# hsp-iit/roft

Measured on AMD Instinct MI355X. Metric: tracker frames/sec per object (640x480) + ADD-S vs CPU ref, higher is better.
Workload: dtype f64; 1 GPU; BASELINE config #4: 640x480, CV_32FC2 flow grid 1, 64 objects in total, 64 per GPU (sharded by object, no data-path collective; result rows all-gathered over RCCL at N > 1), masks+poses at 5 fps with 6-frame delay, flow-aided masks, re-sync and outlier rejection on, frames submitted in batches of at most 8; objects_per_gpu=64, objects_total=64, width=640, height=480, batch_frames=8, ranks=1, backend=nccl

## Files before the change

include/roft_engine.h:

```cpp
#ifndef ROFT_ENGINE_H
#define ROFT_ENGINE_H

#include <stddef.h>
#include <stdint.h>

#ifdef __cplusplus
extern "C" {
#endif

#define ROFT_ABI_VERSION 2

#define ROFT_OK 0
#define ROFT_ERR_INVALID (-1)
#define ROFT_ERR_DEVICE (-2)
#define ROFT_ERR_CAPACITY (-3)
#define ROFT_ERR_STATE (-4)

#define ROFT_FLOW_S16C2 11
#define ROFT_FLOW_F32C2 13

#define ROFT_MEAS_NONE 0
#define ROFT_MEAS_VELOCITY 1
#define ROFT_MEAS_POSE 2
#define ROFT_MEAS_POSE_VELOCITY 3
// ... 250 lines not shown
typedef struct roft_scene_renderer roft_scene_renderer;
int roft_scene_renderer_create(const roft_camera* cam, const roft_mesh* meshes, int n_meshes, int max_frames_per_call, int device,
                               roft_scene_renderer** out);
int roft_scene_renderer_destroy(roft_scene_renderer* r);
int roft_scene_render(roft_scene_renderer* r, const roft_scene_desc* desc, uint8_t* rgb_out, float* depth_out, int32_t* instance_out,
                      int32_t* triangle_out);
int roft_render_scene(const roft_camera* cam, const roft_mesh* meshes, int n_meshes, const roft_scene_desc* desc, uint8_t* rgb_out,
                      float* depth_out, int32_t* instance_out, int32_t* triangle_out);

int roft_debug_plan(const roft_config* cfg, const int* pose_valid, int n_frames, int* n_steps, int* n_corrections,
                    int* outlier, int* slots);
int roft_debug_probe_streams(roft_engine* e, double out[25]);
int roft_debug_sector_rate(int device, double* sectors_per_second);
int roft_debug_get_residency(roft_engine* e, unsigned long long out[32]);
int roft_debug_outlier_split(int mode);
int roft_debug_pose_errors_kernel_ms(double* ms_out);
int roft_debug_scene_kernel_ms(roft_scene_renderer* r, double ms_out[2]);
int roft_debug_get_dbg(roft_engine* e, int obj_id, long long out[32]);

#ifdef __cplusplus
}
#endif
#endif
```

roft_amd/_lib.py:

```python
import ctypes as C
import os
import subprocess

_HERE = os.path.dirname(os.path.abspath(__file__))
CSRC = os.path.join(_HERE, "csrc")
SO = os.environ.get("ROFT_LIB_SO") or os.path.join(CSRC, "libroft_hip.so")

OK = 0
FLOW_S16C2 = 11
FLOW_F32C2 = 13
MEAS_NONE, MEAS_VELOCITY, MEAS_POSE, MEAS_POSE_VELOCITY = 0, 1, 2, 3
MEM_HOST, MEM_DEVICE = 0, 1
RETAIN_FRAMES = 16
MAX_BATCH_FRAMES = 8
MAX_FLOW_CHASE = 30
RENDER_CONTRACT, RENDER_GL = 0, 1
ABI_VERSION = 2


class RoftError(RuntimeError):
    pass


class Camera(C.Structure):
# ... 73 lines not shown


SCENE_MAX_INSTANCES = 256

ABI_SYMBOLS = [
    "roft_last_error_string", "roft_device_count", "roft_abi_version", "roft_flow_measurement", "roft_kf_predict",
    "roft_skf_correct", "roft_skf_correct_points", "roft_mask_propagate", "roft_pose_process_noise", "roft_ukf_predict",
    "roft_ukf_correct", "roft_mesh_classify", "roft_render_depth", "roft_render_depth_mode", "roft_depth_likelihood", "roft_outlier_test",
    "roft_outlier_test_split", "roft_outlier_test_mode", "roft_default_config",
    "roft_default_object", "roft_engine_create", "roft_engine_destroy", "roft_object_add",
    "roft_frame_submit", "roft_frames_submit", "roft_engine_retain_frames", "roft_engine_get_stats", "roft_step", "roft_sync", "roft_get_state", "roft_get_outputs", "roft_get_mask",
    "roft_engine_enable_log", "roft_engine_get_log", "roft_engine_get_log_rows", "roft_engine_stream", "roft_engine_enable_timing",
    "roft_engine_get_timing", "roft_engine_get_batch_trace", "roft_default_of_params", "roft_optical_flow", "roft_flow_producer_create",
    "roft_flow_producer_destroy", "roft_flow_producer_run", "roft_flow_producer_sync", "roft_flow_producer_stream",
    "roft_debug_plan", "roft_debug_get_dbg", "roft_debug_probe_streams", "roft_debug_sector_rate",
    "roft_host_alloc", "roft_host_free", "roft_host_is_pinned", "roft_debug_get_residency", "roft_debug_outlier_split",
    "roft_pose_errors", "roft_engine_score_log", "roft_debug_pose_errors_kernel_ms",
    "roft_scene_renderer_create", "roft_scene_renderer_destroy", "roft_scene_render", "roft_render_scene", "roft_debug_scene_kernel_ms",
]
POSE_ERROR_ADD, POSE_ERROR_ADDS = 0, 1
NEWER_SYMBOLS = ("roft_pose_errors", "roft_engine_score_log", "roft_scene_renderer_create", "roft_scene_renderer_destroy", "roft_scene_render",
                 "roft_render_scene")


def build(force=False):
    srcs = [os.path.join(CSRC, f) for f in os.listdir(CSRC) if f.endswith((".hip", ".h"))]
    srcs.append(os.path.join(_HERE, "..", "include", "roft_engine.h"))
    stale = (not os.path.exists(SO)) or any(os.path.getmtime(s) > os.path.getmtime(SO) for s in srcs)
    if force or stale:
        jobs = str(min(8, os.cpu_count() or 1))
        r = subprocess.run(["make", "-C", CSRC, "-j", jobs, "libroft_hip.so"], capture_output=True, text=True)
# ... 103 lines not shown
```

roft_amd/csrc/engine.hip:

```cpp
#include "engine_internal.h"

namespace {
thread_local std::string g_last_error;
}

namespace roft {
namespace host {
int fail(int code, const std::string& msg)
{
    g_last_error = msg;
    return code;
}
}
}
const std::string& last_error() { return g_last_error; }

namespace roft {
int set_last_error(int code, const std::string& msg) { return fail(code, msg); }

int device_cu_count()
{
    static std::mutex mu;
    static std::vector<int> cus;
    int dev = 0;
// ... 536 lines not shown
    auto bail = [&](int code, const std::string& msg) { delete o; return fail(code, msg); };
    if (d->mesh.n_verts > 0 && d->mesh.n_tris > 0) {
        if (!d->mesh.verts || !d->mesh.tris) return bail(ROFT_ERR_INVALID, "mesh: null vertex or triangle array");
        for (size_t i = 0; i < (size_t)3 * d->mesh.n_tris; ++i)
            if (d->mesh.tris[i] < 0 || d->mesh.tris[i] >= d->mesh.n_verts)
                return bail(ROFT_ERR_INVALID, "mesh: triangle " + std::to_string(i / 3) + " refers to vertex " + std::to_string(d->mesh.tris[i]) +
                                                  " of " + std::to_string(d->mesh.n_verts));
        PreparedMesh pm;
        if (e->cfg.render_mode == ROFT_RENDER_CONTRACT) prepare_mesh(d->mesh.verts, d->mesh.n_verts, d->mesh.tris, d->mesh.n_tris, pm);
        hipError_t err = o->verts.ensure((size_t)3 * d->mesh.n_verts);
        if (err == hipSuccess) err = o->tris.ensure((size_t)3 * d->mesh.n_tris);
        if (err == hipSuccess && pm.closed) err = o->tri_flip.ensure((size_t)d->mesh.n_tris);
        if (err == hipSuccess) err = hipMemcpy(o->verts.p, d->mesh.verts, sizeof(float) * 3 * d->mesh.n_verts, hipMemcpyHostToDevice);
        if (err == hipSuccess) err = hipMemcpy(o->tris.p, pm.tris(d->mesh.tris), sizeof(int32_t) * 3 * d->mesh.n_tris, hipMemcpyHostToDevice);
        if (err == hipSuccess && pm.closed) err = hipMemcpy(o->tri_flip.p, pm.flip.data(), (size_t)d->mesh.n_tris, hipMemcpyHostToDevice);
        if (err != hipSuccess) return bail(ROFT_ERR_DEVICE, std::string("mesh upload: ") + hipGetErrorString(err));
        p.verts = o->verts.p; p.tris = o->tris.p;
        p.tri_flip = pm.closed ? o->tri_flip.p : nullptr;
        p.n_verts = d->mesh.n_verts; p.n_tris = d->mesh.n_tris;
    } else if (e->cfg.outlier_rejection && e->cfg.use_pose) {
        return bail(ROFT_ERR_INVALID, "outlier rejection needs a mesh");
    }
    ObjState* st = new ObjState();
    init_state(*st);
    for (int i = 0; i < 6; ++i) { st->v_mean[i] = d->v_mean0[i]; st->v_cov[i * 6 + i] = d->v_cov0_diag[i]; }
    PoseBelief b{};
    for (int i = 0; i < 13; ++i) b.mean[i] = d->p_mean0[i];
    for (int i = 0; i < 12; ++i) b.cov[i * 12 + i] = d->p_cov0_diag[i];
    st->belief[B_LIN0] = b;
    st->belief[B_LIN1] = b;
    st->belief[B_PRED] = st->belief[B_PRED + 1] = b;
    hipError_t err = hipMemcpy(e->arr.params.p + id, &p, sizeof(p), hipMemcpyHostToDevice);
    if (err == hipSuccess) err = hipMemcpy(e->arr.state.p + id, st, sizeof(ObjState), hipMemcpyHostToDevice);
// ... 13 lines not shown
```

roft_amd/csrc/engine_debug.hip:

```cpp
#include "engine_internal.h"


extern "C" int roft_debug_get_dbg(roft_engine* e, int id, long long out[32])
{
    if (!e || id < 0 || id >= (int)e->objs.size()) return ROFT_ERR_INVALID;
    if (roft_sync(e) != ROFT_OK) return ROFT_ERR_DEVICE;
    ObjState* st = new ObjState();
    hipError_t err = hipMemcpy(st, e->arr.state.p + id, sizeof(ObjState), hipMemcpyDeviceToHost);
    if (err == hipSuccess) std::memcpy(out, st->dbg, sizeof(long long) * 32);
    delete st;
    if (err == hipSuccess) err = hipMemset(reinterpret_cast<char*>(e->arr.state.p + id) + offsetof(ObjState, dbg), 0, sizeof(long long) * 32);
    return err == hipSuccess ? ROFT_OK : ROFT_ERR_DEVICE;
}

extern "C" int roft_debug_outlier_split(int mode)
{
    roft::set_outlier_split(mode);
    return ROFT_OK;
}

extern "C" int roft_debug_get_residency(roft_engine* e, unsigned long long out[32])
{
    if (!e || !out) return ROFT_ERR_INVALID;
    if (roft_sync(e) != ROFT_OK) return ROFT_ERR_DEVICE;
    if (hipMemcpy(out, e->arr.residency.p, sizeof(unsigned long long) * 32, hipMemcpyDeviceToHost) != hipSuccess) return ROFT_ERR_DEVICE;
    return hipMemset(e->arr.residency.p, 0, sizeof(unsigned long long) * 32) == hipSuccess ? ROFT_OK : ROFT_ERR_DEVICE;
}

extern "C" int roft_debug_sector_rate(int device, double* sectors_per_second)
{
    if (!sectors_per_second) return fail(ROFT_ERR_INVALID, "null output");
    HIP_TRY(hipSetDevice(device));
// ... 83 lines not shown
```

roft_amd/csrc/engine_internal.h:

```cpp
#pragma once

#include <hip/hip_runtime.h>

#include <algorithm>
#include <cfloat>
#include <chrono>
#include <cmath>
#include <cstdio>
#include <cstdlib>
#include <cstring>
#include <deque>
#include <map>
#include <mutex>
#include <string>
#include <vector>

#include "roft_device.h"
#include "mesh_class.h"
#include "batch_plan.h"

static_assert(roft::host::kPlanLanes == roft::kNumLin, "batch_plan.h plans for the engine's pose lanes");


namespace roft {
// ... 201 lines not shown
    Sched() { for (int& u : feat_use) u = -1; }
};

struct OwnedFlow {
    DevBuf<unsigned char> buf;
    int last_ref_frame = -1;
};

struct HostObject {
    Sched s;
    int stepped_slot = 0, stepped_lane = 0;
    std::vector<OwnedFlow*> owned;
    DevBuf<float> verts;
    DevBuf<int32_t> tris;
    DevBuf<uint8_t> tri_flip;
    ~HostObject() { for (auto* o : owned) delete o; }
};

struct StageFrame {
    std::vector<DevBuf<unsigned char>*> chunks;
    size_t cur = 0, used = 0;
    std::vector<std::pair<const void*, void*>> seen;
    StageFrame() = default;
    StageFrame(StageFrame&&) = default;
    StageFrame(const StageFrame&) = delete;
    ~StageFrame() { for (auto* c : chunks) delete c; }
};
constexpr size_t kStageChunk = (size_t)32 << 20;


// ... 127 lines not shown
```

roft_amd/csrc/engine_ops.hip:

```cpp
#include "engine_internal.h"

namespace {

struct OpCtx {
    std::mutex mu;
    hipStream_t stream = nullptr;
    Arrays arr;
    int W = 0, H = 0, ftype = 0, fgrid = 0, radius = 0;
    DevBuf<unsigned char> b0, b1, b2, b3, b4, b5, bflip;
    bool ready = false;

    int prepare(const roft_camera& cam, int ftype_, int fgrid_, float fscale, int radius_)
    {
        if (roft_device_count() <= 0) return fail(ROFT_ERR_DEVICE, "no HIP device (libroft_hip has no CPU path)");
        if (int rc = check_geometry(cam.width, cam.height)) return rc;
        HIP_TRY(hipSetDevice(0));
        (void)hipGetLastError();
        if (!stream) HIP_TRY(hipStreamCreateWithFlags(&stream, hipStreamNonBlocking));
        DevFlowFmt ff;
        ff.type = ftype_;
        ff.grid = std::max(fgrid_, 1);
        ff.cols = cam.width / ff.grid;
        ff.rows = cam.height / ff.grid;
        ff.scale = fscale;
// ... 398 lines not shown
    if (int rc = c.arr.ensure_zmerge(1, tpix)) return rc;
    auto restore = [&]() {
        a.cam = make_cam(*cam);
        a.tile_w = cam->width / a.cam.divider;
        a.tile_h = cam->height / a.cam.divider;
        a.max_verts = a.max_tris = 0;
    };
    for (size_t i = 0; i < (size_t)3 * mesh->n_tris; ++i)
        if (mesh->tris[i] < 0 || mesh->tris[i] >= mesh->n_verts) return fail(ROFT_ERR_INVALID, "mesh: a triangle refers to a vertex outside the vertex array");
    PreparedMesh pm;
    if (o_in.render_mode == ROFT_RENDER_CONTRACT) prepare_mesh(mesh->verts, mesh->n_verts, mesh->tris, mesh->n_tris, pm);
    if (int rc = to_dev(c.b0, mesh->verts, (size_t)3 * mesh->n_verts, c.stream)) return rc;
    if (int rc = to_dev(c.b1, pm.tris(mesh->tris), (size_t)3 * mesh->n_tris, c.stream)) return rc;
    if (pm.closed)
        if (int rc = to_dev(c.bflip, pm.flip.data(), (size_t)mesh->n_tris, c.stream)) return rc;
    ObjParams prm;
    std::memset(&prm, 0, sizeof(prm));
    prm.verts = reinterpret_cast<const float*>(c.b0.p);
    prm.tris = reinterpret_cast<const int32_t*>(c.b1.p);
    prm.tri_flip = pm.closed ? reinterpret_cast<const uint8_t*>(c.bflip.p) : nullptr;
    prm.n_verts = mesh->n_verts;
    prm.n_tris = mesh->n_tris;
    a.max_verts = mesh->n_verts;
    a.max_tris = mesh->n_tris;
    FrameCtrl fc;
    clear_ctrl(fc);
    fc.n_steps = 1;
    fc.outlier_step = 0;
    fc.cur_slot = B_LIN0;
    fc.lane = 0;
    fc.feat_read = 0;
    if (depth && mask) {
        std::vector<uint8_t> zero;
        if (int rc = to_dev(c.b2, mask, npix, c.stream)) return rc;
        if (int rc = to_dev(c.b3, depth, npix, c.stream)) return rc;
// ... 211 lines not shown
```

roft_amd/csrc/k_render.hip:

```cpp
#include <algorithm>
#include <atomic>

#include "plane_rank.h"
#include "raster.h"

namespace roft {

constexpr int kFeatThreads = 1024;

#ifdef ROFT_FEAT_PROFILE
#define FTICK(i) do { __syncthreads(); if (threadIdx.x == 0) { long long _t = wall_clock64(); a.state[obj].dbg[i] = _t - f_t0; f_t0 = _t; } } while (0)
#else
#define FTICK(i) do {} while (0)
#endif

template <bool LDS>
__global__ __launch_bounds__(kFeatThreads) void features_kernel(EngineArrays a, unsigned frames_packed)
{
    ROFT_RESIDENT(a, RK_FEATURES);
    extern __shared__ __attribute__((aligned(16))) unsigned char smem[];
    __shared__ int s_wave[16];
    __shared__ int s_chunk[kFeatThreads];
    const int obj = blockIdx.x;
    const FrameCtrl& c = frame_ctrl(a, (int)((frames_packed >> (4 * blockIdx.y)) & 15u), obj);
// ... 279 lines not shown
    const int alt = bx / parts, part = bx % parts, tid = threadIdx.x;
    ObjState& st = a.state[obj];
    PoseLane& pl = st.lane[lin];
    if (pl.pending_frame < 0) return;
    const FrameCtrl& c = frame_ctrl(a, pl.pending_frame, obj);
    const ObjParams& prm = a.params[obj];
    const PoseBelief& bl = st.belief[b_alt(lin, alt)];
    const RenderPose P = make_pose(bl.mean + 6, bl.mean + 9);
    const int d = a.cam.divider, tw = a.tile_w, th = a.tile_h;
    const float fx = (float)(a.cam.fx / d), fy = (float)(a.cam.fy / d), cx = (float)(a.cam.cx / d), cy = (float)(a.cam.cy / d);
    const int nv = prm.n_verts, nt = prm.n_tris;
    const bool cached = nv <= vcache_cap;
    float* s_v = reinterpret_cast<float*>(smem);
    uint32_t* s_z = reinterpret_cast<uint32_t*>(smem + (((size_t)vcache_cap * 12 + 15) & ~(size_t)15));
    uint64_t* s_k = reinterpret_cast<uint64_t*>(s_z);
    if (tid < 4) s_box[tid] = (tid < 2) ? INT32_MAX : -1;
    if (tid == 0) s_behind = 0;
#ifdef ROFT_FUSED_PROFILE
    long long u_t0 = wall_clock64();
    if (tid < 8 && bx < 4) st.dbg[bx * 8 + tid] = 0;
#endif
    __syncthreads();
    {
        int bi0 = INT32_MAX, bj0 = INT32_MAX, bi1 = -1, bj1 = -1;
        bool behind = false;
        constexpr int kVB = 4;
        for (int vb = tid; vb < nv; vb += kVB * kFusedThreads) {
          float vc[kVB][3];
#pragma unroll
          for (int k = 0; k < kVB; ++k) {
// ... 23 lines not shown
        for (int off = 32; off > 0; off >>= 1) {
            bi0 = min(bi0, __shfl_xor(bi0, off, 64)); bj0 = min(bj0, __shfl_xor(bj0, off, 64));
            bi1 = max(bi1, __shfl_xor(bi1, off, 64)); bj1 = max(bj1, __shfl_xor(bj1, off, 64));
        }
        if ((tid & 63) == 0) {
            atomicMin(&s_box[0], bi0); atomicMin(&s_box[1], bj0);
            atomicMax(&s_box[2], bi1); atomicMax(&s_box[3], bj1);
        }
    }
    __syncthreads();
    UTICK(0);
    const int i0 = min(s_box[0], tw - 1), i1 = s_box[2];
    int j0 = min(s_box[1], th - 1), j1 = s_box[3];
    int R = parts;
    if (!GL && split_tris && parts > 1 && i1 >= i0 && j1 >= j0 && i0 >= 0 && j0 >= 0) {
        const long long w_all = i1 - i0 + 1, rows_all = j1 - j0 + 1;
        for (R = 1; R < parts; ++R)
            if (parts % R == 0 && ((rows_all + R - 1) / R) * w_all <= (long long)win_cap) break;
    }
    const int G = parts / R, band = part / G, grp = part % G;
    const bool split = G > 1;
    if (j1 >= j0 && R > 1) {
        const int rows_all = j1 - j0 + 1, b0 = j0 + (int)((long long)rows_all * band / R), b1 = j0 + (int)((long long)rows_all * (band + 1) / R) - 1;
        j0 = b0;
        j1 = b1;
    }
    const int win_w = i1 - i0 + 1;
    const int fslot = (c.feat_read >= 0) ? c.feat_read : 0;
    const uint32_t* fpix = a.feat_pix + ((size_t)obj * kFeatRing + fslot) * a.feat_cap;
    const float* fdep = a.feat_depth + ((size_t)obj * kFeatRing + fslot) * a.feat_cap;
    const int n = st.n_feat[fslot];
    LikelihoodSum err;
    int cnt = 0;
    auto gl_resolve = [&](uint64_t key, int i, int j) -> float {
        const int32_t* tri = prm.tris + (size_t)3 * (uint32_t)key;
        const int v0 = tri[0], v1 = tri[1], v2 = tri[2];
        float x0, y0, z0, x1, y1, z1, x2, y2, z2;
        if (cached) {
// ... 2 lines not shown
            x2 = s_v[3 * v2]; y2 = s_v[3 * v2 + 1]; z2 = s_v[3 * v2 + 2];
        } else {
            project_vertex_gl(prm.verts + (size_t)3 * v0, P, fx, fy, cx, cy, x0, y0, z0);
            project_vertex_gl(prm.verts + (size_t)3 * v1, P, fx, fy, cx, cy, x1, y1, z1);
            project_vertex_gl(prm.verts + (size_t)3 * v2, P, fx, fy, cx, cy, x2, y2, z2);
        }
        return gl_linear_depth(gl_pixel_window_z(x0, y0, x1, y1, x2, y2, gl_vertex_window_z(z0), gl_vertex_window_z(z1),
                                                 gl_vertex_window_z(z2), (float)i + 0.5f, (float)j + 0.5f));
    };
    if (win_w > 0 && j1 >= j0 && i0 >= 0 && j0 >= 0) {
        const int rows = max(1, win_cap / win_w);
        for (int js = j0; js <= j1; js += rows) {
            const int je = min(j1, js + rows - 1), npx = win_w * (je - js + 1);
            if constexpr (GL) {
                for (int i = tid; i < npx; i += kFusedThreads) s_k[i] = kGlKeyClear;
            } else {
                for (int i = tid; i < npx; i += kFusedThreads) s_z[i] = 0x7F800000u;
            }
            __syncthreads();
            UTICK(1);
            ROFT_LDS uint32_t* const zw = pin_lds(s_z);
            auto store = [zw, i0, js, win_w](int i, int j, float z) {
                (void)__hip_atomic_fetch_min(zw + ((j - js) * win_w + (i - i0)), __float_as_uint(z), __ATOMIC_RELAXED, __HIP_MEMORY_SCOPE_WORKGROUP);
            };
            ROFT_LDS uint64_t* const zk = (ROFT_LDS uint64_t*)zw;
            auto store_key = [zk, i0, js, win_w](int i, int j, uint64_t key) {
                (void)__hip_atomic_fetch_min(zk + ((j - js) * win_w + (i - i0)), key, __ATOMIC_RELAXED, __HIP_MEMORY_SCOPE_WORKGROUP);
            };
            constexpr int kTB = 8;
            const uint8_t* const flips = (!GL && prm.tri_flip && !s_behind && nv < (1 << 30)) ? prm.tri_flip : nullptr;
            const int stride = G, first = grp;
            auto tri_of = [=](int slot) { return ((slot >> 6) * stride + first) * 64 + (slot & 63); };
            const int n_slots = split ? ((nt + 63) / 64 + stride - 1 - first) / stride * 64 : nt;
            for (int tb = tid; tb < n_slots; tb += kTB * kFusedThreads) {
              int idx[kTB][3];
#pragma unroll
              for (int k = 0; k < kTB; ++k) {
                  const int t = min(tri_of(min(tb + k * kFusedThreads, n_slots - 1)), nt - 1);
                  const int32_t* tri = prm.tris + (size_t)3 * t;
                  idx[k][0] = tri[0]; idx[k][1] = tri[1]; idx[k][2] = tri[2];
                  if (flips) idx[k][0] |= (1 + (int)flips[t]) << 30;
              }
#pragma unroll
              for (int k = 0; k < kTB; ++k) {
                if (tb + k * kFusedThreads >= n_slots || tri_of(tb + k * kFusedThreads) >= nt) break;
                const int cull_k = (int)((unsigned)idx[k][0] >> 30);
                const int v0 = idx[k][0] & 0x3FFFFFFF, v1 = idx[k][1], v2 = idx[k][2];
                float x0, y0, z0, x1, y1, z1, x2, y2, z2;
                if (cached) {
                    x0 = s_v[3 * v0]; y0 = s_v[3 * v0 + 1]; z0 = s_v[3 * v0 + 2];
                    x1 = s_v[3 * v1]; y1 = s_v[3 * v1 + 1]; z1 = s_v[3 * v1 + 2];
                    x2 = s_v[3 * v2]; y2 = s_v[3 * v2 + 1]; z2 = s_v[3 * v2 + 2];
                } else if constexpr (GL) {
                    project_vertex_gl(prm.verts + (size_t)3 * v0, P, fx, fy, cx, cy, x0, y0, z0);
                    project_vertex_gl(prm.verts + (size_t)3 * v1, P, fx, fy, cx, cy, x1, y1, z1);
                    project_vertex_gl(prm.verts + (size_t)3 * v2, P, fx, fy, cx, cy, x2, y2, z2);
                } else {
                    project_vertex(prm.verts + (size_t)3 * v0, P, fx, fy, cx, cy, x0, y0, z0);
                    project_vertex(prm.verts + (size_t)3 * v1, P, fx, fy, cx, cy, x1, y1, z1);
                    project_vertex(prm.verts + (size_t)3 * v2, P, fx, fy, cx, cy, x2, y2, z2);
                }
                if constexpr (GL) {
                    const uint64_t t = (uint32_t)tri_of(tb + k * kFusedThreads);
                    raster_projected_gl(x0, y0, z0, x1, y1, z1, x2, y2, z2, tw, th, js, je,
                                        [&](int i, int j, uint32_t qz) { store_key(i, j, ((uint64_t)qz << 32) | t); });
                } else {
                    raster_projected(x0, y0, z0, x1, y1, z1, x2, y2, z2, tw, th, js, je, cull_k, store);
                }
              }
            }
            __syncthreads();
            UTICK(2);
            if constexpr (!GL) if (split) {
                const size_t slab0 = (((size_t)lin * a.zmerge_slabs + (size_t)obj * parts + (size_t)band * G) * 2 + alt) * a.zmerge_stride;
                uint32_t* mine = a.zmerge + slab0 + (size_t)grp * 2 * a.zmerge_stride;
                int* arrivals = a.zcount + (((size_t)lin * a.n_obj + obj) * 2 + alt) * kMaxOutlierParts + band;
                for (int i = tid; i < npx; i += kFusedThreads)
                    __hip_atomic_store(&mine[i], s_z[i], __ATOMIC_RELAXED, __HIP_MEMORY_SCOPE_AGENT);
                __atomic_signal_fence(__ATOMIC_SEQ_CST);
                __builtin_amdgcn_s_waitcnt(0);
                __atomic_signal_fence(__ATOMIC_SEQ_CST);
                __syncthreads();
                if (tid == 0) {
                    const int before = __hip_atomic_fetch_add(arrivals, 1, __ATOMIC_RELAXED, __HIP_MEMORY_SCOPE_AGENT);
                    s_last = (before == G - 1) ? 1 : 0;
                    if (before == G - 1) __hip_atomic_store(arrivals, 0, __ATOMIC_RELAXED, __HIP_MEMORY_SCOPE_AGENT);
                }
                __syncthreads();
                if (!s_last) return;
                static_assert(kMaxOutlierParts <= 8, "eight slabs per pixel");
                const uint32_t* others = a.zmerge + slab0;
                const size_t slab_step = 2 * a.zmerge_stride;
                const uint32_t* op[7];
                {
                    int k = 0;
#pragma unroll
                    for (int p = 0; p < 8; ++p)
                        if (p < G && p != grp && k < 7) op[k++] = others + (size_t)p * slab_step;
                    for (; k < 7; ++k) op[k] = others;
                }
                for (int i = tid; i < npx; i += kFusedThreads) {
                    uint32_t m = s_z[i];
                    uint32_t v0, v1, v2, v3, v4, v5, v6;
                    switch (G - 1) {
                    case 1:
                        asm volatile("global_load_dword %0, %1, off sc1\n\ts_waitcnt vmcnt(0)" : "=&v"(v0) : "v"(op[0] + i) : "memory");
                        m = min(m, v0);
                        break;
                    case 2:
                        asm volatile("global_load_dword %0, %2, off sc1\n\tglobal_load_dword %1, %3, off sc1\n\ts_waitcnt vmcnt(0)"
                                     : "=&v"(v0), "=&v"(v1) : "v"(op[0] + i), "v"(op[1] + i) : "memory");
                        m = min(m, min(v0, v1));
                        break;
                    case 3:
                        asm volatile("global_load_dword %0, %3, off sc1\n\tglobal_load_dword %1, %4, off sc1\n\tglobal_load_dword %2, %5, off sc1\n\t"
                                     "s_waitcnt vmcnt(0)"
                                     : "=&v"(v0), "=&v"(v1), "=&v"(v2) : "v"(op[0] + i), "v"(op[1] + i), "v"(op[2] + i) : "memory");
                        m = min(min(m, v0), min(v1, v2));
                        break;
                    case 4:
                        asm volatile("global_load_dword %0, %4, off sc1\n\tglobal_load_dword %1, %5, off sc1\n\tglobal_load_dword %2, %6, off sc1\n\t"
                                     "global_load_dword %3, %7, off sc1\n\ts_waitcnt vmcnt(0)"
                                     : "=&v"(v0), "=&v"(v1), "=&v"(v2), "=&v"(v3) : "v"(op[0] + i), "v"(op[1] + i), "v"(op[2] + i), "v"(op[3] + i) : "memory");
                        m = min(m, min(min(v0, v1), min(v2, v3)));
                        break;
                    default:
                        asm volatile("global_load_dword %0, %7, off sc1\n\tglobal_load_dword %1, %8, off sc1\n\tglobal_load_dword %2, %9, off sc1\n\t"
                                     "global_load_dword %3, %10, off sc1\n\tglobal_load_dword %4, %11, off sc1\n\tglobal_load_dword %5, %12, off sc1\n\t"
                                     "global_load_dword %6, %13, off sc1\n\ts_waitcnt vmcnt(0)"
                                     : "=&v"(v0), "=&v"(v1), "=&v"(v2), "=&v"(v3), "=&v"(v4), "=&v"(v5), "=&v"(v6)
                                     : "v"(op[0] + i), "v"(op[1] + i), "v"(op[2] + i), "v"(op[3] + i), "v"(op[4] + i), "v"(op[5] + i), "v"(op[6] + i) : "memory");
                        m = min(min(m, v0), min(min(v1, v2), min(min(v3, v4), min(v5, v6))));
                        break;
                    case 0: break;
                    }
                    s_z[i] = m;
                }
                __syncthreads();
            }
            if (tile_dump) {
                float* tile = tile_dump + (size_t)alt * tw * th;
                if constexpr (GL) {
                    for (int i = tid; i < npx; i += kFusedThreads) {
                        const uint64_t key = s_k[i];
                        const int pi = i0 + i % win_w, pj = js + i / win_w;
                        tile[(size_t)pj * tw + pi] = ((uint32_t)(key >> 32) == kGlDepthClear) ? 0.0f : gl_resolve(key, pi, pj);
                    }
                } else {
                    for (int i = tid; i < npx; i += kFusedThreads) {
                        const uint32_t b = s_z[i];
                        tile[(size_t)(js + i / win_w) * tw + (i0 + i % win_w)] = (b == 0x7F800000u) ? 0.0f : __uint_as_float(b);
                    }
                }
            }
            constexpr int kBatch = 16;
            for (int f0 = tid; f0 < n; f0 += kBatch * kFusedThreads) {
                float dep[kBatch];
                uint32_t pix[kBatch];
#pragma unroll
                for (int k = 0; k < kBatch; ++k) {
                    const int i = f0 + k * kFusedThreads;
                    dep[k] = (i < n) ? fdep[i] : 0.0f;
                    pix[k] = (i < n) ? fpix[i] : 0u;
                }
#pragma unroll
                for (int k = 0; k < kBatch; ++k) {
                    if (!((dep[k] > 0) && ((double)dep[k] < 2.0))) continue;
                    const int v = (int)(pix[k] >> 16), u = (int)(pix[k] & 0xFFFFu);
                    const int tj = v / d, ti = u / d;
                    if (tj < js || tj > je || ti < i0 || ti > i1) continue;
// ... 24 lines not shown
    __syncthreads();
    if (tid == 0) {
        long long hi = 0, lo = 0;
        int n2 = 0;
        for (int w = 0; w < kFusedThreads / 64; ++w) { hi += s_hi[w]; lo += s_lo[w]; n2 += s_cnt[w]; }
        pl.part_hi[alt][band] = hi;
        pl.part_lo[alt][band] = lo;
        pl.part_cnt[alt][band] = (double)n2;
        if (band == 0) pl.n_parts[alt] = R;
    }
}

static std::atomic<int> g_outlier_split{-1};
void set_outlier_split(int mode) { g_outlier_split.store(mode < 0 ? -1 : (mode ? 1 : 0), std::memory_order_relaxed); }

void launch_outlier(const EngineArrays& a, int lin, hipStream_t s, hipEvent_t stop, const OutlierLaunchOpts* opts)
{
    const size_t lds_total = 160 * 1024 - 4096;
    const size_t vbytes = ((size_t)a.max_verts * 12 + 15) & ~(size_t)15;
    const bool gl = opts && opts->render_mode == ROFT_RENDER_GL;
    const size_t zb = gl ? 8 : 4;
    const size_t min_win = zb * std::max(8192, a.tile_w);
    const bool cache = vbytes + min_win <= lds_total && !(opts && opts->no_vertex_cache);
    const int vcache_cap = cache ? a.max_verts : 0;
    int win_cap = (int)((lds_total - (cache ? vbytes : 0)) / zb);
    (void)set_max_dynamic_lds(gl ? reinterpret_cast<const void*>(outlier_fused_kernel<true>) : reinterpret_cast<const void*>(outlier_fused_kernel<false>),
                              (int)lds_total);
    int parts = std::max(1, std::min(kMaxOutlierParts, device_cu_count() / (2 * std::max(a.n_obj, 1))));
    if (a.outlier_parts > 0) parts = std::min(a.outlier_parts, kMaxOutlierParts);
    if (opts && opts->parts > 0) parts = std::min(opts->parts, kMaxOutlierParts);
    if (opts && opts->parts < 0) parts = std::max(1, parts / -opts->parts);
    static const int split_env = getenv("ROFT_OUTLIER_SPLIT") ? atoi(getenv("ROFT_OUTLIER_SPLIT")) : -1;
    const int forced = g_outlier_split.load(std::memory_order_relaxed) >= 0 ? g_outlier_split.load(std::memory_order_relaxed) : split_env;
// ... 23 lines not shown
```

roft_amd/csrc/mesh_class.h:

```cpp
#pragma once

#include <cstdint>
#include <vector>

namespace roft {

bool classify_mesh(const float* verts, int n_verts, const int32_t* tris, int n_tris, std::vector<uint8_t>& flip);

void facing_coherent_order(const float* verts, const int32_t* tris, int n_tris, const std::vector<uint8_t>& flip, std::vector<int32_t>& order);

struct PreparedMesh {
    bool closed = false;
    std::vector<int32_t> reordered;
    std::vector<uint8_t> flip;
    const int32_t* tris(const int32_t* callers) const { return closed ? reordered.data() : callers; }
};
void prepare_mesh(const float* verts, int n_verts, const int32_t* tris, int n_tris, PreparedMesh& out);

}
```

roft_amd/csrc/mesh_class.hip:

```cpp
#include "mesh_class.h"

#include <algorithm>
#include <cmath>
#include <cstring>
#include <numeric>

namespace roft {

bool classify_mesh(const float* verts, int n_verts, const int32_t* tris, int n_tris, std::vector<uint8_t>& flip)
{
    flip.assign((size_t)std::max(n_tris, 0), 0);
    if (n_verts <= 0 || n_tris <= 0) return false;
    struct P { float x, y, z; };
    std::vector<P> pos((size_t)n_verts);
    for (int i = 0; i < n_verts; ++i) {
        pos[i] = {verts[3 * i] + 0.0f, verts[3 * i + 1] + 0.0f, verts[3 * i + 2] + 0.0f};
        if (std::isnan(pos[i].x) || std::isnan(pos[i].y) || std::isnan(pos[i].z)) return false;
    }
    std::vector<int> by_pos((size_t)n_verts), id((size_t)n_verts);
    std::iota(by_pos.begin(), by_pos.end(), 0);
    std::sort(by_pos.begin(), by_pos.end(), [&](int a, int b) {
        if (pos[a].x != pos[b].x) return pos[a].x < pos[b].x;
        if (pos[a].y != pos[b].y) return pos[a].y < pos[b].y;
        if (pos[a].z != pos[b].z) return pos[a].z < pos[b].z;
// ... 86 lines not shown
        if (std::fabs(n[1]) > std::fabs(n[ax])) ax = 1;
        if (std::fabs(n[2]) > std::fabs(n[ax])) ax = 2;
        const int face = 2 * ax + (n[ax] < 0.0 ? 1 : 0), u = (ax + 1) % 3, v = (ax + 2) % 3;
        key[t] = face * 4 + (n[u] < 0.0 ? 1 : 0) * 2 + (n[v] < 0.0 ? 1 : 0);
        order[t] = t;
    }
    std::stable_sort(order.begin(), order.end(), [&](int32_t a, int32_t b) { return key[a] < key[b]; });
}

void prepare_mesh(const float* verts, int n_verts, const int32_t* tris, int n_tris, PreparedMesh& out)
{
    std::vector<uint8_t> flip;
    out.closed = classify_mesh(verts, n_verts, tris, n_tris, flip);
    out.reordered.clear();
    out.flip.clear();
    if (!out.closed) return;
    std::vector<int32_t> order;
    facing_coherent_order(verts, tris, n_tris, flip, order);
    out.reordered.resize((size_t)3 * n_tris);
    out.flip.resize((size_t)n_tris);
    for (int k = 0; k < n_tris; ++k) {
        const int32_t t = order[k];
        for (int q = 0; q < 3; ++q) out.reordered[(size_t)3 * k + q] = tris[(size_t)3 * t + q];
        out.flip[k] = flip[t];
    }
}

}
```

roft_amd/csrc/roft_device.h:

```cpp
#pragma once

#include <hip/hip_runtime.h>
#include <hip/hip_ext.h>
#include <stdint.h>

#include "../../include/roft_engine.h"

namespace roft {

constexpr int kWave = 64;
constexpr int kNumLin = 2;
constexpr int kNumBelief = 9;
constexpr int kMaxBatch = ROFT_MAX_BATCH_FRAMES;
constexpr int kTwistRing = 64;
constexpr int kMaxFlowHist = ROFT_MAX_FLOW_CHASE;
constexpr int kMaxOutlierParts = 8;
constexpr int kMaxSteps = 10;
constexpr int kPlaneSlots = 64;
constexpr int kFeatRing = 12;

enum BeliefSlot { B_LIN0 = 0, B_LIN1 = 1, B_PRED = 2 , B_ALT0 = 4 , B_ALT1 = 5 ,
                  B_SPARE = 8, B_CORR = B_LIN0  };
__host__ __device__ inline int b_alt(int lane, int k) { return B_ALT0 + 2 * lane + k; }

// ... 14 lines not shown
    double mean[13];
    double cov[144];
};

struct ObjParams {
    double sigma_ang_vel[3];
    double psd_lin_acc[3];
    double v_q[6];
    double R_v[3], R_w[3], R_x[3], R_q[3];
    double r_flow[2];
    const float* verts;
    const int32_t* tris;
    int n_verts, n_tris;
    const double* q_override;
    const uint8_t* tri_flip;
};

struct FlowRec {
    int u, v;
    float z, dx, dy;
};

struct PoseLane {
    int pc_frame, pc_step;
    int pending_frame;
    int outlier_selected;
    double outlier_L[2];
    double outlier_cnt[2];
    int ukf_status;
    int n_parts[2];
// ... 243 lines not shown
                        const double* Rdiag, int reweight, double* norms, double* x_out, double* P_out, int* status,
                        hipStream_t s);
void launch_kf_predict(const double* x, const double* P, const double* qdiag, double* xo, double* Po, hipStream_t s);
void launch_ukf_chain(const EngineArrays& a, roft_ut_params ut, bool first_segment, int lin, hipStream_t s, hipEvent_t stop = nullptr);
void launch_features(const EngineArrays& a, hipStream_t s, hipEvent_t stop = nullptr, unsigned feat_frames = 0);
struct OutlierLaunchOpts {
    int parts = 0;
    int no_vertex_cache = 0;
    int window_pixels = 0;
    float* tile_dump = nullptr;
    int split = -1;
    int render_mode = ROFT_RENDER_CONTRACT;
};
void launch_outlier(const EngineArrays& a, int lin, hipStream_t s, hipEvent_t stop = nullptr, const OutlierLaunchOpts* opts = nullptr);
void set_outlier_split(int mode);
void launch_outlier_only(const EngineArrays& a, hipStream_t s);

int device_cu_count();
hipError_t set_max_dynamic_lds(const void* func, int bytes);

void launch_expand_yh(const FlowRec* recs, const int* n, DevCamera cam, double dt, int32_t* uv, double* y,
                      double* H, int cap, hipStream_t s);

constexpr int kCandBatch = 8;
struct PoseView {
    const double* base;
    long stride;
    int first, ring;
};
int pose_error_padded_points(int P);
// ... 7 lines not shown
```

Before: 1.697 million object-frames/s.

## Pack triangles into 64-bit records and vectorize outlier depth slab merge

Adds a host-side packing of each triangle's three vertex indices plus a cull code into one 64-bit record, uploaded at object creation. The outlier raster kernel fetches these with one global load per triangle, using a software-prefetched loop, instead of three index loads plus a flip-byte load. The kernel also clears the depth window once with vector stores, merges the cross-part z slabs with dwordx4 loads through scalar base pointers, and shrinks several batch sizes and the LDS budget. The goals are less memory traffic and fewer instructions per triangle and per pixel. In exchange it adds packing state, a 20-bit vertex limit that falls back to the old path, and more complex merge code.

```diff
diff --git a/include/roft_engine.h b/include/roft_engine.h
--- a/include/roft_engine.h
+++ b/include/roft_engine.h
@@ -288,6 +288,8 @@
 int roft_debug_sector_rate(int device, double* sectors_per_second);
 int roft_debug_get_residency(roft_engine* e, unsigned long long out[32]);
 int roft_debug_outlier_split(int mode);
+int roft_debug_outlier_tri_records(int on);
+int roft_debug_outlier_tri_record_uploads(long* count_out);
 int roft_debug_pose_errors_kernel_ms(double* ms_out);
 int roft_debug_scene_kernel_ms(roft_scene_renderer* r, double ms_out[2]);
 int roft_debug_get_dbg(roft_engine* e, int obj_id, long long out[32]);
diff --git a/roft_amd/_lib.py b/roft_amd/_lib.py
--- a/roft_amd/_lib.py
+++ b/roft_amd/_lib.py
@@ -111,7 +111,7 @@
     "roft_engine_get_timing", "roft_engine_get_batch_trace", "roft_default_of_params", "roft_optical_flow", "roft_flow_producer_create",
     "roft_flow_producer_destroy", "roft_flow_producer_run", "roft_flow_producer_sync", "roft_flow_producer_stream",
     "roft_debug_plan", "roft_debug_get_dbg", "roft_debug_probe_streams", "roft_debug_sector_rate",
-    "roft_host_alloc", "roft_host_free", "roft_host_is_pinned", "roft_debug_get_residency", "roft_debug_outlier_split",
+    "roft_host_alloc", "roft_host_free", "roft_host_is_pinned", "roft_debug_get_residency", "roft_debug_outlier_split", "roft_debug_outlier_tri_records", "roft_debug_outlier_tri_record_uploads",
     "roft_pose_errors", "roft_engine_score_log", "roft_debug_pose_errors_kernel_ms",
     "roft_scene_renderer_create", "roft_scene_renderer_destroy", "roft_scene_render", "roft_render_scene", "roft_debug_scene_kernel_ms",
 ]
diff --git a/roft_amd/csrc/engine.hip b/roft_amd/csrc/engine.hip
--- a/roft_amd/csrc/engine.hip
+++ b/roft_amd/csrc/engine.hip
@@ -574,9 +574,14 @@
         if (err == hipSuccess) err = hipMemcpy(o->verts.p, d->mesh.verts, sizeof(float) * 3 * d->mesh.n_verts, hipMemcpyHostToDevice);
         if (err == hipSuccess) err = hipMemcpy(o->tris.p, pm.tris(d->mesh.tris), sizeof(int32_t) * 3 * d->mesh.n_tris, hipMemcpyHostToDevice);
         if (err == hipSuccess && pm.closed) err = hipMemcpy(o->tri_flip.p, pm.flip.data(), (size_t)d->mesh.n_tris, hipMemcpyHostToDevice);
+        const bool packed = !pm.packed.empty() && outlier_tri_records();
+        if (err == hipSuccess && packed) err = o->tri_pack.ensure(pm.packed.size());
+        if (err == hipSuccess && packed) err = hipMemcpy(o->tri_pack.p, pm.packed.data(), sizeof(uint64_t) * pm.packed.size(), hipMemcpyHostToDevice);
         if (err != hipSuccess) return bail(ROFT_ERR_DEVICE, std::string("mesh upload: ") + hipGetErrorString(err));
         p.verts = o->verts.p; p.tris = o->tris.p;
         p.tri_flip = pm.closed ? o->tri_flip.p : nullptr;
+        p.tri_pack = packed ? o->tri_pack.p : nullptr;
+        if (packed) note_tri_record_upload();
         p.n_verts = d->mesh.n_verts; p.n_tris = d->mesh.n_tris;
     } else if (e->cfg.outlier_rejection && e->cfg.use_pose) {
         return bail(ROFT_ERR_INVALID, "outlier rejection needs a mesh");
diff --git a/roft_amd/csrc/engine_debug.hip b/roft_amd/csrc/engine_debug.hip
--- a/roft_amd/csrc/engine_debug.hip
+++ b/roft_amd/csrc/engine_debug.hip
@@ -16,6 +16,19 @@
 extern "C" int roft_debug_outlier_split(int mode)
 {
     roft::set_outlier_split(mode);
+    return ROFT_OK;
+}
+
+extern "C" int roft_debug_outlier_tri_records(int on)
+{
+    roft::set_outlier_tri_records(on);
+    return ROFT_OK;
+}
+
+extern "C" int roft_debug_outlier_tri_record_uploads(long* count_out)
+{
+    if (!count_out) return ROFT_ERR_INVALID;
+    *count_out = roft::tri_record_uploads();
     return ROFT_OK;
 }
 
diff --git a/roft_amd/csrc/engine_internal.h b/roft_amd/csrc/engine_internal.h
--- a/roft_amd/csrc/engine_internal.h
+++ b/roft_amd/csrc/engine_internal.h
@@ -239,6 +239,7 @@
     DevBuf<float> verts;
     DevBuf<int32_t> tris;
     DevBuf<uint8_t> tri_flip;
+    DevBuf<uint64_t> tri_pack;
     ~HostObject() { for (auto* o : owned) delete o; }
 };
 
diff --git a/roft_amd/csrc/engine_ops.hip b/roft_amd/csrc/engine_ops.hip
--- a/roft_amd/csrc/engine_ops.hip
+++ b/roft_amd/csrc/engine_ops.hip
@@ -7,7 +7,7 @@
     hipStream_t stream = nullptr;
     Arrays arr;
     int W = 0, H = 0, ftype = 0, fgrid = 0, radius = 0;
-    DevBuf<unsigned char> b0, b1, b2, b3, b4, b5, bflip;
+    DevBuf<unsigned char> b0, b1, b2, b3, b4, b5, bflip, bpack;
     bool ready = false;
 
     int prepare(const roft_camera& cam, int ftype_, int fgrid_, float fscale, int radius_)
@@ -436,11 +436,16 @@
     if (int rc = to_dev(c.b1, pm.tris(mesh->tris), (size_t)3 * mesh->n_tris, c.stream)) return rc;
     if (pm.closed)
         if (int rc = to_dev(c.bflip, pm.flip.data(), (size_t)mesh->n_tris, c.stream)) return rc;
+    const bool packed = !pm.packed.empty() && outlier_tri_records();
+    if (packed)
+        if (int rc = to_dev(c.bpack, pm.packed.data(), pm.packed.size(), c.stream)) return rc;
     ObjParams prm;
     std::memset(&prm, 0, sizeof(prm));
     prm.verts = reinterpret_cast<const float*>(c.b0.p);
     prm.tris = reinterpret_cast<const int32_t*>(c.b1.p);
     prm.tri_flip = pm.closed ? reinterpret_cast<const uint8_t*>(c.bflip.p) : nullptr;
+    prm.tri_pack = packed ? reinterpret_cast<const uint64_t*>(c.bpack.p) : nullptr;
+    if (packed) note_tri_record_upload();
     prm.n_verts = mesh->n_verts;
     prm.n_tris = mesh->n_tris;
     a.max_verts = mesh->n_verts;
diff --git a/roft_amd/csrc/k_render.hip b/roft_amd/csrc/k_render.hip
--- a/roft_amd/csrc/k_render.hip
+++ b/roft_amd/csrc/k_render.hip
@@ -3,6 +3,7 @@
 
 #include "plane_rank.h"
 #include "raster.h"
+#include "tri_pack.h"
 
 namespace roft {
 
@@ -317,6 +318,13 @@
     float* s_v = reinterpret_cast<float*>(smem);
     uint32_t* s_z = reinterpret_cast<uint32_t*>(smem + (((size_t)vcache_cap * 12 + 15) & ~(size_t)15));
     uint64_t* s_k = reinterpret_cast<uint64_t*>(s_z);
+    if constexpr (!GL) {
+        typedef uint32_t u32x4 __attribute__((ext_vector_type(4)));
+        u32x4* const z4 = reinterpret_cast<u32x4*>(s_z);
+        const u32x4 empty = {0x7F800000u, 0x7F800000u, 0x7F800000u, 0x7F800000u};
+        for (int i = tid; i < (win_cap >> 2); i += kFusedThreads) z4[i] = empty;
+        if (tid < (win_cap & 3)) s_z[(win_cap & ~3) + tid] = 0x7F800000u;
+    }
     if (tid < 4) s_box[tid] = (tid < 2) ? INT32_MAX : -1;
     if (tid == 0) s_behind = 0;
 #ifdef ROFT_FUSED_PROFILE
@@ -370,14 +378,15 @@
     int j0 = min(s_box[1], th - 1), j1 = s_box[3];
     int R = parts;
     if (!GL && split_tris && parts > 1 && i1 >= i0 && j1 >= j0 && i0 >= 0 && j0 >= 0) {
-        const long long w_all = i1 - i0 + 1, rows_all = j1 - j0 + 1;
+        const uint32_t w_all = (uint32_t)(i1 - i0 + 1), rows_all = (uint32_t)(j1 - j0 + 1);
         for (R = 1; R < parts; ++R)
-            if (parts % R == 0 && ((rows_all + R - 1) / R) * w_all <= (long long)win_cap) break;
+            if ((uint32_t)parts % (uint32_t)R == 0 && ((rows_all + (uint32_t)R - 1) / (uint32_t)R) * w_all <= (uint32_t)win_cap) break;
     }
     const int G = parts / R, band = part / G, grp = part % G;
     const bool split = G > 1;
     if (j1 >= j0 && R > 1) {
-        const int rows_all = j1 - j0 + 1, b0 = j0 + (int)((long long)rows_all * band / R), b1 = j0 + (int)((long long)rows_all * (band + 1) / R) - 1;
+        const uint32_t rows_all = (uint32_t)(j1 - j0 + 1);
+        const int b0 = j0 + (int)(rows_all * (uint32_t)band / (uint32_t)R), b1 = j0 + (int)(rows_all * (uint32_t)(band + 1) / (uint32_t)R) - 1;
         j0 = b0;
         j1 = b1;
     }
@@ -410,10 +419,11 @@
             const int je = min(j1, js + rows - 1), npx = win_w * (je - js + 1);
             if constexpr (GL) {
                 for (int i = tid; i < npx; i += kFusedThreads) s_k[i] = kGlKeyClear;
-            } else {
+                __syncthreads();
+            } else if (js != j0) {
                 for (int i = tid; i < npx; i += kFusedThreads) s_z[i] = 0x7F800000u;
+                __syncthreads();
             }
-            __syncthreads();
             UTICK(1);
             ROFT_LDS uint32_t* const zw = pin_lds(s_z);
             auto store = [zw, i0, js, win_w](int i, int j, float z) {
@@ -423,25 +433,11 @@
             auto store_key = [zk, i0, js, win_w](int i, int j, uint64_t key) {
                 (void)__hip_atomic_fetch_min(zk + ((j - js) * win_w + (i - i0)), key, __ATOMIC_RELAXED, __HIP_MEMORY_SCOPE_WORKGROUP);
             };
-            constexpr int kTB = 8;
-            const uint8_t* const flips = (!GL && prm.tri_flip && !s_behind && nv < (1 << 30)) ? prm.tri_flip : nullptr;
+            const bool culling = !GL && prm.tri_flip && !s_behind;
             const int stride = G, first = grp;
             auto tri_of = [=](int slot) { return ((slot >> 6) * stride + first) * 64 + (slot & 63); };
             const int n_slots = split ? ((nt + 63) / 64 + stride - 1 - first) / stride * 64 : nt;
-            for (int tb = tid; tb < n_slots; tb += kTB * kFusedThreads) {
-              int idx[kTB][3];
-#pragma unroll
-              for (int k = 0; k < kTB; ++k) {
-                  const int t = min(tri_of(min(tb + k * kFusedThreads, n_slots - 1)), nt - 1);
-                  const int32_t* tri = prm.tris + (size_t)3 * t;
-                  idx[k][0] = tri[0]; idx[k][1] = tri[1]; idx[k][2] = tri[2];
-                  if (flips) idx[k][0] |= (1 + (int)flips[t]) << 30;
-              }
-#pragma unroll
-              for (int k = 0; k < kTB; ++k) {
-                if (tb + k * kFusedThreads >= n_slots || tri_of(tb + k * kFusedThreads) >= nt) break;
-                const int cull_k = (int)((unsigned)idx[k][0] >> 30);
-                const int v0 = idx[k][0] & 0x3FFFFFFF, v1 = idx[k][1], v2 = idx[k][2];
+            auto draw = [&](int slot, int v0, int v1, int v2, int cull_k) {
                 float x0, y0, z0, x1, y1, z1, x2, y2, z2;
                 if (cached) {
                     x0 = s_v[3 * v0]; y0 = s_v[3 * v0 + 1]; z0 = s_v[3 * v0 + 2];
@@ -457,13 +453,57 @@
                     project_vertex(prm.verts + (size_t)3 * v2, P, fx, fy, cx, cy, x2, y2, z2);
                 }
                 if constexpr (GL) {
-                    const uint64_t t = (uint32_t)tri_of(tb + k * kFusedThreads);
+                    const uint64_t t = (uint32_t)tri_of(slot);
                     raster_projected_gl(x0, y0, z0, x1, y1, z1, x2, y2, z2, tw, th, js, je,
                                         [&](int i, int j, uint32_t qz) { store_key(i, j, ((uint64_t)qz << 32) | t); });
                 } else {
                     raster_projected(x0, y0, z0, x1, y1, z1, x2, y2, z2, tw, th, js, je, cull_k, store);
                 }
-              }
+            };
+            typedef const __attribute__((address_space(1))) uint64_t* GlobalRecords;
+            const GlobalRecords recs = GL ? nullptr : (GlobalRecords)prm.tri_pack;
+            if (recs) {
+                constexpr int kTR = 2;
+                uint32_t lo[kTR], hi[kTR];
+                auto fetch = [&](int tb) {
+#pragma unroll
+                    for (int k = 0; k < kTR; ++k) {
+                        const int t = min(tri_of(min(tb + k * kFusedThreads, n_slots - 1)), nt - 1);
+                        const uint64_t w = recs[t];
+                        lo[k] = (uint32_t)w; hi[k] = (uint32_t)(w >> 32);
+                    }
+                };
+                if (tid < n_slots) fetch(tid);
+                for (int tb = tid; tb < n_slots; tb += kTR * kFusedThreads) {
+                    uint32_t clo[kTR], chi[kTR];
+#pragma unroll
+                    for (int k = 0; k < kTR; ++k) { clo[k] = lo[k]; chi[k] = hi[k]; }
+                    if (tb + kTR * kFusedThreads < n_slots) fetch(tb + kTR * kFusedThreads);
+#pragma unroll
+                    for (int k = 0; k < kTR; ++k) {
+                        if (tb + k * kFusedThreads >= n_slots || tri_of(tb + k * kFusedThreads) >= nt) break;
+                        const host::TriRecord r = host::tri_unpack(clo[k], chi[k]);
+                        draw(tb + k * kFusedThreads, (int)r.v0, (int)r.v1, (int)r.v2, culling ? (int)r.cull : 0);
+                    }
+                }
+            } else {
+                constexpr int kTB = GL ? 8 : 2;
+                const uint8_t* const flips = (culling && nv < (1 << 30)) ? prm.tri_flip : nullptr;
+                for (int tb = tid; tb < n_slots; tb += kTB * kFusedThreads) {
+                    int idx[kTB][3];
+#pragma unroll
+                    for (int k = 0; k < kTB; ++k) {
+                        const int t = min(tri_of(min(tb + k * kFusedThreads, n_slots - 1)), nt - 1);
+                        const int32_t* tri = prm.tris + (size_t)3 * t;
+                        idx[k][0] = tri[0]; idx[k][1] = tri[1]; idx[k][2] = tri[2];
+                        if (flips) idx[k][0] |= (1 + (int)flips[t]) << 30;
+                    }
+#pragma unroll
+                    for (int k = 0; k < kTB; ++k) {
+                        if (tb + k * kFusedThreads >= n_slots || tri_of(tb + k * kFusedThreads) >= nt) break;
+                        draw(tb + k * kFusedThreads, idx[k][0] & 0x3FFFFFFF, idx[k][1], idx[k][2], (int)((unsigned)idx[k][0] >> 30));
+                    }
+                }
             }
             __syncthreads();
             UTICK(2);
@@ -484,7 +524,8 @@
                 }
                 __syncthreads();
                 if (!s_last) return;
-                static_assert(kMaxOutlierParts <= 8, "eight slabs per pixel");
+                static_assert(kMaxOutlierParts <= 8, "seven other slabs per block");
+                typedef uint32_t u32x4 __attribute__((ext_vector_type(4)));
                 const uint32_t* others = a.zmerge + slab0;
                 const size_t slab_step = 2 * a.zmerge_stride;
                 const uint32_t* op[7];
@@ -494,42 +535,57 @@
                     for (int p = 0; p < 8; ++p)
                         if (p < G && p != grp && k < 7) op[k++] = others + (size_t)p * slab_step;
                     for (; k < 7; ++k) op[k] = others;
-                }
-                for (int i = tid; i < npx; i += kFusedThreads) {
-                    uint32_t m = s_z[i];
-                    uint32_t v0, v1, v2, v3, v4, v5, v6;
+                    for (k = 0; k < 7; ++k) {
+                        const uint64_t v = reinterpret_cast<uint64_t>(op[k]);
+                        const uint32_t lo = __builtin_amdgcn_readfirstlane((uint32_t)v), hi = __builtin_amdgcn_readfirstlane((uint32_t)(v >> 32));
+                        op[k] = reinterpret_cast<const uint32_t*>(((uint64_t)hi << 32) | lo);
+                    }
+                }
+                auto min4 = [](u32x4 x, u32x4 y) { return __builtin_elementwise_min(x, y); };
+                u32x4* const z4 = reinterpret_cast<u32x4*>(s_z);
+                const int n_blocks = (a.zmerge_stride & 3) ? 0 : npx >> 2;
+                for (int q = tid; q < n_blocks; q += kFusedThreads) {
+                    const uint32_t off = (uint32_t)q * 16u;
+                    u32x4 m = z4[q];
+                    u32x4 v0, v1, v2, v3, v4, v5, v6;
                     switch (G - 1) {
                     case 1:
-                        asm volatile("global_load_dword %0, %1, off sc1\n\ts_waitcnt vmcnt(0)" : "=&v"(v0) : "v"(op[0] + i) : "memory");
-                        m = min(m, v0);
+                        asm volatile("global_load_dwordx4 %0, %1, %2 sc1\n\ts_waitcnt vmcnt(0)" : "=&v"(v0) : "v"(off), "s"(op[0]) : "memory");
+                        m = min4(m, v0);
                         break;
                     case 2:
-                        asm volatile("global_load_dword %0, %2, off sc1\n\tglobal_load_dword %1, %3, off sc1\n\ts_waitcnt vmcnt(0)"
-                                     : "=&v"(v0), "=&v"(v1) : "v"(op[0] + i), "v"(op[1] + i) : "memory");
-                        m = min(m, min(v0, v1));
+                        asm volatile("global_load_dwordx4 %0, %2, %3 sc1\n\tglobal_load_dwordx4 %1, %2, %4 sc1\n\ts_waitcnt vmcnt(0)"
+                                     : "=&v"(v0), "=&v"(v1) : "v"(off), "s"(op[0]), "s"(op[1]) : "memory");
+                        m = min4(m, min4(v0, v1));
                         break;
                     case 3:
-                        asm volatile("global_load_dword %0, %3, off sc1\n\tglobal_load_dword %1, %4, off sc1\n\tglobal_load_dword %2, %5, off sc1\n\t"
+                        asm volatile("global_load_dwordx4 %0, %3, %4 sc1\n\tglobal_load_dwordx4 %1, %3, %5 sc1\n\tglobal_load_dwordx4 %2, %3, %6 sc1\n\t"
                                      "s_waitcnt vmcnt(0)"
-                                     : "=&v"(v0), "=&v"(v1), "=&v"(v2) : "v"(op[0] + i), "v"(op[1] + i), "v"(op[2] + i) : "memory");
-                        m = min(min(m, v0), min(v1, v2));
+                                     : "=&v"(v0), "=&v"(v1), "=&v"(v2) : "v"(off), "s"(op[0]), "s"(op[1]), "s"(op[2]) : "memory");
+                        m = min4(min4(m, v0), min4(v1, v2));
                         break;
                     case 4:
-                        asm volatile("global_load_dword %0, %4, off sc1\n\tglobal_load_dword %1, %5, off sc1\n\tglobal_load_dword %2, %6, off sc1\n\t"
-                                     "global_load_dword %3, %7, off sc1\n\ts_waitcnt vmcnt(0)"
-                                     : "=&v"(v0), "=&v"(v1), "=&v"(v2), "=&v"(v3) : "v"(op[0] + i), "v"(op[1] + i), "v"(op[2] + i), "v"(op[3] + i) : "memory");
-                        m = min(m, min(min(v0, v1), min(v2, v3)));
+                        asm volatile("global_load_dwordx4 %0, %4, %5 sc1\n\tglobal_load_dwordx4 %1, %4, %6 sc1\n\tglobal_load_dwordx4 %2, %4, %7 sc1\n\t"
+                                     "global_load_dwordx4 %3, %4, %8 sc1\n\ts_waitcnt vmcnt(0)"
+                                     : "=&v"(v0), "=&v"(v1), "=&v"(v2), "=&v"(v3) : "v"(off), "s"(op[0]), "s"(op[1]), "s"(op[2]), "s"(op[3]) : "memory");
+                        m = min4(m, min4(min4(v0, v1), min4(v2, v3)));
                         break;
                     default:
-                        asm volatile("global_load_dword %0, %7, off sc1\n\tglobal_load_dword %1, %8, off sc1\n\tglobal_load_dword %2, %9, off sc1\n\t"
-                                     "global_load_dword %3, %10, off sc1\n\tglobal_load_dword %4, %11, off sc1\n\tglobal_load_dword %5, %12, off sc1\n\t"
-                                     "global_load_dword %6, %13, off sc1\n\ts_waitcnt vmcnt(0)"
+                        asm volatile("global_load_dwordx4 %0, %7, %8 sc1\n\tglobal_load_dwordx4 %1, %7, %9 sc1\n\tglobal_load_dwordx4 %2, %7, %10 sc1\n\t"
+                                     "global_load_dwordx4 %3, %7, %11 sc1\n\tglobal_load_dwordx4 %4, %7, %12 sc1\n\tglobal_load_dwordx4 %5, %7, %13 sc1\n\t"
+                                     "global_load_dwordx4 %6, %7, %14 sc1\n\ts_waitcnt vmcnt(0)"
                                      : "=&v"(v0), "=&v"(v1), "=&v"(v2), "=&v"(v3), "=&v"(v4), "=&v"(v5), "=&v"(v6)
-                                     : "v"(op[0] + i), "v"(op[1] + i), "v"(op[2] + i), "v"(op[3] + i), "v"(op[4] + i), "v"(op[5] + i), "v"(op[6] + i) : "memory");
-                        m = min(min(m, v0), min(min(v1, v2), min(min(v3, v4), min(v5, v6))));
+                                     : "v"(off), "s"(op[0]), "s"(op[1]), "s"(op[2]), "s"(op[3]), "s"(op[4]), "s"(op[5]), "s"(op[6]) : "memory");
+                        m = min4(min4(m, v0), min4(min4(v1, v2), min4(min4(v3, v4), min4(v5, v6))));
                         break;
                     case 0: break;
                     }
+                    z4[q] = m;
+                }
+                for (int i = 4 * n_blocks + tid; i < npx; i += kFusedThreads) {
+                    uint32_t m = s_z[i];
+                    for (int p = 0; p < G; ++p)
+                        if (p != grp) m = min(m, __hip_atomic_load(others + (size_t)p * slab_step + i, __ATOMIC_RELAXED, __HIP_MEMORY_SCOPE_AGENT));
                     s_z[i] = m;
                 }
                 __syncthreads();
@@ -549,7 +605,7 @@
                     }
                 }
             }
-            constexpr int kBatch = 16;
+            constexpr int kBatch = GL ? 16 : 8;
             for (int f0 = tid; f0 < n; f0 += kBatch * kFusedThreads) {
                 float dep[kBatch];
                 uint32_t pix[kBatch];
@@ -604,9 +660,16 @@
 static std::atomic<int> g_outlier_split{-1};
 void set_outlier_split(int mode) { g_outlier_split.store(mode < 0 ? -1 : (mode ? 1 : 0), std::memory_order_relaxed); }
 
+static std::atomic<int> g_tri_records{1};
+void set_outlier_tri_records(int on) { g_tri_records.store(on ? 1 : 0, std::memory_order_relaxed); }
+bool outlier_tri_records() { return g_tri_records.load(std::memory_order_relaxed) != 0; }
+static std::atomic<long> g_tri_record_uploads{0};
+void note_tri_record_upload() { g_tri_record_uploads.fetch_add(1, std::memory_order_relaxed); }
+long tri_record_uploads() { return g_tri_record_uploads.load(std::memory_order_relaxed); }
+
 void launch_outlier(const EngineArrays& a, int lin, hipStream_t s, hipEvent_t stop, const OutlierLaunchOpts* opts)
 {
-    const size_t lds_total = 160 * 1024 - 4096;
+    const size_t lds_total = 160 * 1024 - 12 * 1024 - 1024;
     const size_t vbytes = ((size_t)a.max_verts * 12 + 15) & ~(size_t)15;
     const bool gl = opts && opts->render_mode == ROFT_RENDER_GL;
     const size_t zb = gl ? 8 : 4;
diff --git a/roft_amd/csrc/mesh_class.h b/roft_amd/csrc/mesh_class.h
--- a/roft_amd/csrc/mesh_class.h
+++ b/roft_amd/csrc/mesh_class.h
@@ -2,6 +2,8 @@
 
 #include <cstdint>
 #include <vector>
+
+#include "tri_pack.h"
 
 namespace roft {
 
@@ -13,6 +15,7 @@
     bool closed = false;
     std::vector<int32_t> reordered;
     std::vector<uint8_t> flip;
+    std::vector<uint64_t> packed;
     const int32_t* tris(const int32_t* callers) const { return closed ? reordered.data() : callers; }
 };
 void prepare_mesh(const float* verts, int n_verts, const int32_t* tris, int n_tris, PreparedMesh& out);
diff --git a/roft_amd/csrc/mesh_class.hip b/roft_amd/csrc/mesh_class.hip
--- a/roft_amd/csrc/mesh_class.hip
+++ b/roft_amd/csrc/mesh_class.hip
@@ -124,15 +124,21 @@
     out.closed = classify_mesh(verts, n_verts, tris, n_tris, flip);
     out.reordered.clear();
     out.flip.clear();
-    if (!out.closed) return;
-    std::vector<int32_t> order;
-    facing_coherent_order(verts, tris, n_tris, flip, order);
-    out.reordered.resize((size_t)3 * n_tris);
-    out.flip.resize((size_t)n_tris);
-    for (int k = 0; k < n_tris; ++k) {
-        const int32_t t = order[k];
-        for (int q = 0; q < 3; ++q) out.reordered[(size_t)3 * k + q] = tris[(size_t)3 * t + q];
-        out.flip[k] = flip[t];
+    out.packed.clear();
+    if (out.closed) {
+        std::vector<int32_t> order;
+        facing_coherent_order(verts, tris, n_tris, flip, order);
+        out.reordered.resize((size_t)3 * n_tris);
+        out.flip.resize((size_t)n_tris);
+        for (int k = 0; k < n_tris; ++k) {
+            const int32_t t = order[k];
+            for (int q = 0; q < 3; ++q) out.reordered[(size_t)3 * k + q] = tris[(size_t)3 * t + q];
+            out.flip[k] = flip[t];
+        }
+    }
+    if (host::tri_pack_fits(n_verts) && n_tris > 0) {
+        out.packed.resize((size_t)n_tris);
+        host::tri_pack_mesh(out.tris(tris), out.closed ? out.flip.data() : nullptr, n_verts, n_tris, out.packed.data());
     }
 }
 
diff --git a/roft_amd/csrc/roft_device.h b/roft_amd/csrc/roft_device.h
--- a/roft_amd/csrc/roft_device.h
+++ b/roft_amd/csrc/roft_device.h
@@ -52,6 +52,7 @@
     int n_verts, n_tris;
     const double* q_override;
     const uint8_t* tri_flip;
+    const uint64_t* tri_pack;
 };
 
 struct FlowRec {
@@ -325,6 +326,10 @@
 };
 void launch_outlier(const EngineArrays& a, int lin, hipStream_t s, hipEvent_t stop = nullptr, const OutlierLaunchOpts* opts = nullptr);
 void set_outlier_split(int mode);
+void set_outlier_tri_records(int on);
+bool outlier_tri_records();
+void note_tri_record_upload();
+long tri_record_uploads();
 void launch_outlier_only(const EngineArrays& a, hipStream_t s);
 
 int device_cu_count();
diff --git a/roft_amd/csrc/tri_pack.h b/roft_amd/csrc/tri_pack.h
--- /dev/null
+++ b/roft_amd/csrc/tri_pack.h
@@ -0,0 +1,41 @@
+#pragma once
+
+#include <cstddef>
+#include <cstdint>
+
+namespace roft {
+namespace host {
+
+constexpr int kTriPackIndexBits = 20;
+constexpr int kTriPackMaxVerts = 1 << kTriPackIndexBits;
+
+constexpr bool tri_pack_fits(int n_verts) { return n_verts > 0 && n_verts < kTriPackMaxVerts; }
+
+constexpr uint32_t tri_cull_code(bool closed, uint32_t flip) { return closed ? 1u + (flip ? 1u : 0u) : 0u; }
+
+constexpr uint64_t tri_pack(uint32_t v0, uint32_t v1, uint32_t v2, uint32_t cull)
+{
+    return (uint64_t)(v0 & 0xFFFFFu) | ((uint64_t)(v1 & 0xFFFFFu) << 20) | ((uint64_t)(v2 & 0xFFFFFu) << 40) | ((uint64_t)(cull & 3u) << 60);
+}
+
+struct TriRecord {
+    uint32_t v0, v1, v2, cull;
+};
+
+constexpr TriRecord tri_unpack(uint32_t lo, uint32_t hi)
+{
+    return TriRecord{lo & 0xFFFFFu, (lo >> 20) | ((hi & 0xFFu) << 12), (hi >> 8) & 0xFFFFFu, (hi >> 28) & 3u};
+}
+constexpr TriRecord tri_unpack(uint64_t w) { return tri_unpack((uint32_t)w, (uint32_t)(w >> 32)); }
+
+inline bool tri_pack_mesh(const int32_t* tris, const uint8_t* flip, int n_verts, int n_tris, uint64_t* out)
+{
+    if (!tri_pack_fits(n_verts)) return false;
+    for (int t = 0; t < n_tris; ++t)
+        out[t] = tri_pack((uint32_t)tris[(size_t)3 * t], (uint32_t)tris[(size_t)3 * t + 1], (uint32_t)tris[(size_t)3 * t + 2],
+                          tri_cull_code(flip != nullptr, flip ? flip[t] : 0u));
+    return true;
+}
+
+}
+}
```

After: 1.710 million object-frames/s, median of 4. No clear change (+0.7%).
